# liruihui/SP-GAN

Hardware: AMD Instinct MI355X
Metric: G+D train-step shapes/sec @2048 pts, bs=32 per GPU (WGAN-GP) (higher is better)
Workload: dtype f32; 1 GPU; BASELINE configs[1]: Chair-shaped synthetic clouds, 2048 pts, per-GPU batch 32, WGAN + gradient penalty (lambda 10), 1 D-step + 1 G-step, Adam(1e-4, (0.5,0.99)), k=10; one latent per shape (default noise_generator) handed over un-tiled [b,1,128]; global_batch=32, n_points=2048, parallelism=dp1

## Files before the change

### include/spgan_hip.h

```cpp
#ifndef SPGAN_HIP_H
#define SPGAN_HIP_H

#include <stddef.h>
#include <stdint.h>

#ifdef __cplusplus
extern "C" {
#endif

typedef void* spgan_stream_t;

#define SPGAN_OK 0
#define SPGAN_EINVAL (-22)
#define SPGAN_ECOMM (-70)

int spgan_version(void);
const char* spgan_arch(void);


int spgan_knn(const float* x_pm, int B, int N, int C, int k, int mode, int32_t* idx, spgan_stream_t s);

size_t spgan_knn_ws_bytes(int B, int N, int C, int k, int mode);
int spgan_knn_ws(const float* x_pm, int B, int N, int C, int k, int mode, int32_t* idx, void* ws, size_t ws_bytes, spgan_stream_t s);

// ... 179 lines not shown
size_t spgan_colreduce_ws_bytes(int M, int C, int G);
int spgan_colstats_finalize(const float* partials, int groups, int tiles_per_group, int C, int G, int mode,
                            int tile_rows , float* out0, float* out1, spgan_stream_t s);
int spgan_colstats_finalize_bn(const float* partials, int tiles, int C, int G, int tile_rows, const float* gamma, const float* beta,
                               float eps, float momentum, float* running_mean, float* running_var, float* scale, float* shift,
                               float* invstd, float* mean_out, spgan_stream_t s);
int spgan_colstats_finalize_bn_groups(const float* partials, int groups, int tiles_per_group, int C, int G, int tile_rows, const float* gamma,
                                      const float* beta, float eps, float momentum, float* running_mean, float* running_var, float* out,
                                      spgan_stream_t s);
int spgan_colstats_finalize_bn2(const float* partials, int tiles, int C, int G, int tile_rows, int split, const float* gammaA,
                                const float* betaA, float* rmeanA, float* rvarA, const float* gammaB, const float* betaB, float* rmeanB,
                                float* rvarB, float eps, float momentum, int count_rep, float* out4, spgan_stream_t s);
int spgan_colstats(const float* X, int ldx, int M, int C, int G, float slope, float* out_mean, float* out_var,
                   float* ws, size_t ws_bytes, spgan_stream_t s);
int spgan_colsum(const float* X, int ldx, int M, int C, int G, float* out, float* ws, size_t ws_bytes, spgan_stream_t s);

int spgan_bn_prepare(const float* mean, const float* var, const float* gamma, const float* beta, int C,
                     int count, float eps, float momentum, int training,
                     float* running_mean, float* running_var,
                     float* scale, float* shift, float* invstd, float* mean_used, spgan_stream_t s);
int spgan_bn_bwd_apply(const float* g, const float* y, int ld, int M, int C, const float* mean, const float* invstd,
                       const float* gamma, const float* sums, int count, float* dy, spgan_stream_t s);
int spgan_bn_bwd_apply2(const float* g, const float* g2, const float* g2scale, const float* y, int M, int C, const float* mean,
                        const float* invstd, const float* gamma, const float* sums, int count, float* dy, spgan_stream_t s);

int spgan_maxpool(const float* y, int ld, int B, int N, int C, const float* scale, const float* shift, float slope,
                  float* out, int32_t* argmax, spgan_stream_t s);

int spgan_edge_wcat(const float* Ww0 , const float* Wx , int H, int F, int C, float* Wcat, float* WcatT, spgan_stream_t s);
int spgan_conv_out_weight_pm(const float* w, int F, int k, float* Wo, float* WoT, spgan_stream_t s);
int spgan_edge_wcat_bwd(const float* dWcat, int H, int F, int C, float* dWw0, float* dWx, spgan_stream_t s);
int spgan_edge_stats_tile_rows(int k);
int spgan_edge_stats(const float* PQR, int ld, const int32_t* idx, int M, int k, int H, int F, const float* b1, const float* bx,
                     float* partials, spgan_stream_t s);
int spgan_edge_attend_fwd(const float* h2pre, const float* sc2, const float* sh2, const float* PQR, int ld, int H, int F,
                          const int32_t* idx, int M, int k, const float* bx, const float* scx, const float* shx, float slope,
                          float* T, spgan_stream_t s);
int spgan_edge_attend_fwd_h(const void* h2pre, int h2_half, const float* sc2, const float* sh2, const float* PQR, int ld, int H, int F,
                            const int32_t* idx, int M, int k, const float* bx, const float* scx, const float* shx, float slope, uint16_t* T_f16,
                            spgan_stream_t s);
int spgan_edge_attend_bwd_b(const uint16_t* dT_bf16, const void* h2pre, int h2_half, const float* sc2, const float* sh2, const float* mean2,
                            const float* inv2, const float* PQR, int ld, int H, int F, const int32_t* idx, int M, int k, const float* bx,
                            const float* scx, const float* shx, const float* meanx, const float* invx, float slope, uint16_t* g2_bf16,
                            uint16_t* gy_bf16, float* partials, spgan_stream_t s);
int spgan_edge_scatter_b(const float* g1, const uint16_t* gy_bf16, const float* PQR, int ld, int H, int F, const int32_t* idx,
                         const int32_t* rowptr, const int32_t* src, int M, int k, const float* b1, const float* mean1, const float* inv1,
                         const float* gam1, const float* sums1, const float* bx, const float* meanx, const float* invx, const float* gamx,
                         const float* sumsx, float* dPQR, spgan_stream_t s);
int spgan_edge_attend_bwd_tile_points(void);
int spgan_edge_attend_bwd(const float* dT, const float* h2pre, const float* sc2, const float* sh2, const float* mean2,
                          const float* inv2, const float* PQR, int ld, int H, int F, const int32_t* idx, int M, int k,
                          const float* bx, const float* scx, const float* shx, const float* meanx, const float* invx,
                          float slope, float* g2, float* gy, float* partials, spgan_stream_t s);
int spgan_edge_scatter(const float* g1, const float* gy, const float* PQR, int ld, int H, int F, const int32_t* idx,
                       const int32_t* rowptr, const int32_t* src, int M, int k, const float* b1, const float* mean1,
                       const float* inv1, const float* gam1, const float* sums1, const float* bx, const float* meanx,
                       const float* invx, const float* gamx, const float* sumsx, float* dPQR, spgan_stream_t s);

int spgan_adain_fwd(const float* x, int M, int C, int N, float slope, const float* imean, const float* ivar, float eps,
                    const float* gb, float* out, spgan_stream_t s);
int spgan_adain_bwd1(const float* dout, const float* x, int M, int C, int N, float slope, const float* imean, const float* ivar,
                     float eps, const float* gb, int ld_gamma, long x_shape_stride, float* dgb, float* partials, spgan_stream_t s);
int spgan_adain_bwd2(const float* dout, const float* x, int M, int C, int N, float slope, const float* imean, const float* ivar,
                     float eps, const float* gb, int ld_gamma, long x_shape_stride, const float* S0, const float* S1, float* dx,
                     spgan_stream_t s);

int spgan_pool_bwd_stats(const float* gpool, const float* pooled, const int32_t* argmax, const float* y, int ld, const float* mean,
                         const float* invstd, float slope, int B, int C, float* gval, float* sums , spgan_stream_t s);
int spgan_pool_bwd_stats_prep(const float* gpool, const float* pooled, const int32_t* argmax, const float* y, int ld, const float* mean,
                              const float* invstd, float slope, int B, int C, const float* gamma, int count, float* gval, float* sums ,
                              float* alpha, float* beta, float* cg, spgan_stream_t s);
int spgan_bn_bwd_apply_sparse(const float* gval, const int32_t* argmax, const float* y, int ld, int M, int C, int N,
                              const float* mean, const float* invstd, const float* gamma, const float* sums, int count, float* dy,
                              spgan_stream_t s);
int spgan_maxpool_bwd_add(const float* dpool, const int32_t* argmax, int B, int C, float* dst, int ld, spgan_stream_t s);
int spgan_tanh_bwd(const float* dy, const float* y, size_t n, float* out, spgan_stream_t s);
int spgan_act_bwd(const float* dy, const float* y, size_t n, int act, float slope, float* out, spgan_stream_t s);
int spgan_scatter_rows(const float* val, const int32_t* argmax, int B, int C, int M, float* out, spgan_stream_t s);
int spgan_gather_rows(const float* src, int ld, const int32_t* argmax, int B, int C, float* out, spgan_stream_t s);

int spgan_bn_dbl_stats(const float* u, const float* y, const float* gz, int M, int C, const float* mean, const float* invstd,
                       float* partials, spgan_stream_t s);
int spgan_bn_dbl_apply(const float* u, const float* y, const float* gz, int M, int C, const float* mean, const float* invstd,
                       const float* scale, const float* shift, float slope, const float* gamma, const float* S1, const float* U0,
                       const float* U1, float* q, float* xbar, spgan_stream_t s);
int spgan_gan_loss(int mode, int which, const float* d_real, const float* d_fake, const float* real_label, const float* fake_label,
                   int B, float* out5, float* g_real, float* g_fake, spgan_stream_t s);
int spgan_lerp_rows(const float* real, const float* fake, const float* alpha, int B, size_t L, float* out, spgan_stream_t s);
int spgan_gp_penalty_fwd(const float* g, int B, size_t L, float gamma, float lambda, float* norms, float* loss, spgan_stream_t s);
int spgan_gp_penalty_bwd(const float* g, const float* norms, int B, size_t L, float gamma, float lambda, const float* upstream,
                         float* v, spgan_stream_t s);
int spgan_gp_penalty_fwd_bwd(const float* g, int B, size_t L, float gamma, float lambda, float* norms, float* loss, const float* loss_add,
                             float* loss_total, float* v, spgan_stream_t s);
int spgan_square_distance(const float* src, const float* dst, int B, int N, int M, int C, float* out, spgan_stream_t s);
int spgan_index_points(const float* points, const int64_t* idx, int B, int N, int C, int S, float* out, spgan_stream_t s);
int spgan_farthest_point_sample(const float* xyz, int B, int N, int npoint, const int64_t* start, int64_t* out, float* dist_ws,
                                spgan_stream_t s);
int spgan_query_ball_point(float radius, int nsample, const float* xyz, const float* new_xyz, int B, int N, int S, int C,
                           int64_t* out, spgan_stream_t s);
int spgan_knn_point(int nsample, const float* xyz, const float* new_xyz, int B, int N, int S, int C, int64_t* out, spgan_stream_t s);
int spgan_group_concat(const float* xyz, const float* center, const float* feat, const int64_t* idx, int B, int N, int S, int K,
                       int C, int D, float* out, spgan_stream_t s);
int spgan_gather_csr(const int64_t* idx, int B, int S, int N, int32_t* rowptr, int32_t* src, int32_t* bad, spgan_stream_t s);
int spgan_scatter_slots(const float* dout, int ld, int col0, int C, const int32_t* rowptr, const int32_t* src, int BN, float* dpoints,
                        spgan_stream_t s);
int spgan_group_center_bwd(const float* dout, int ld, int Q, int K, int C, float* dcenter, spgan_stream_t s);
// ... 330 lines not shown
```

### sp-gan_amd/csrc/edge.hip

```cpp
#include <stdlib.h>
#include "common.hpp"

namespace {

__device__ __forceinline__ int xcd_block() {
  const int per = gridDim.x >> 3;
  return (int)(blockIdx.x & 7) * per + (int)(blockIdx.x >> 3);
}
inline int grid8(long n) { return (int)((n + 7) / 8 * 8); }

__global__ void edge_wcat_kernel(const float* __restrict__ Ww0, const float* __restrict__ Wx, int H, int F, int C, float* __restrict__ Wcat,
                                 float* __restrict__ WcatT) {
  const int t = blockIdx.x * blockDim.x + threadIdx.x;
  if (t >= (H + 2 * F) * C) return;
  const int row = t / C, c = t % C;
  float v;
  if (row < H) v = Ww0[row * C + c];
  else if (row < H + F) v = Wx[(row - H) * 2 * C + C + c];
  else v = Wx[(row - H - F) * 2 * C + c] - Wx[(row - H - F) * 2 * C + C + c];
  Wcat[t] = v;
  if (WcatT) WcatT[c * (H + 2 * F) + row] = v;
}
__global__ void conv_out_weight_pm_kernel(const float* __restrict__ w, int F, int k, float* __restrict__ Wo, float* __restrict__ WoT) {
  const int t = blockIdx.x * blockDim.x + threadIdx.x;
  if (t >= F * F * k) return;
  const int o = t / (k * F), q = t % (k * F), r = q / F, c = q % F;
  const float v = w[((size_t)o * F + c) * k + r];
  Wo[t] = v;
  if (WoT) WoT[(size_t)q * F + o] = v;
}
__global__ void edge_wcat_bwd_kernel(const float* __restrict__ dWcat, int H, int F, int C, float* __restrict__ dWw0, float* __restrict__ dWx) {
  const int t = blockIdx.x * blockDim.x + threadIdx.x;
  if (t < H * C) dWw0[t] = dWcat[t];
  if (t < F * C) {
    const int f = t / C, c = t % C;
    const float dq = dWcat[(H + f) * C + c], dr = dWcat[(H + F + f) * C + c];
    dWx[f * 2 * C + c] = dr;
    dWx[f * 2 * C + C + c] = dq - dr;
  }
}

constexpr int ES_PT = 32;

__device__ __forceinline__ float edge_pre(const float* __restrict__ PQR, int ld, int H, int F, int c, int i, int j, float bias) {
  if (c < H) return (PQR[(size_t)j * ld + c] - PQR[(size_t)i * ld + c]) + bias;
  const int f = c - H;
  return (PQR[(size_t)i * ld + H + F + f] + PQR[(size_t)j * ld + H + f]) + bias;
}

template <int KT>
__global__ __launch_bounds__(256) void edge_stats_kernel(const float* __restrict__ PQR, int ld, const int32_t* __restrict__ idx, int M, int k_,
                                                         int H, int F, const float* __restrict__ b1, const float* __restrict__ bx,
                                                         float* __restrict__ part) {
  constexpr int KU = KT > 0 ? KT : 1;
  const int k = KT > 0 ? KT : k_;
  __shared__ float red[4][64];
  const int lane = threadIdx.x & 63, w = __builtin_amdgcn_readfirstlane(threadIdx.x >> 6);
  const int bxid = xcd_block();
  const int p0 = bxid * ES_PT;
  if (p0 >= M) return;
  const int np = min(ES_PT, M - p0);
  const int CH = H + F;
// ... 251 lines not shown
      const float rden = 1.0f / den;
#pragma unroll
      for (int r = 0; r < K; ++r) {
        const float yv = lrelu_f(fmaf((Ri[q] + qv[r][q]) + bb[q], ax[q], cx[q]), slope);
        z[r][q] = yv * (z[r][q] * rden);
      }
    }
#pragma unroll
    for (int r = 0; r < K; ++r) {
      if (TH) stv_h<VEC>(reinterpret_cast<_Float16*>(T) + ((size_t)i * K + r) * F + f, z[r]);
      else stv<VEC>(T + ((size_t)i * K + r) * F + f, z[r]);
    }
  }
}

template <int K, int VEC, int TB = 0, int HH = 0>
__global__ __launch_bounds__(256) void edge_attend_bwd_k_kernel(
    const float* __restrict__ dT, const float* __restrict__ h2, const float* __restrict__ sc2, const float* __restrict__ sh2,
    const float* __restrict__ mean2, const float* __restrict__ inv2, const float* __restrict__ PQR, int ld, int H, int F,
    const int32_t* __restrict__ idx, int M, const float* __restrict__ bx, const float* __restrict__ scx, const float* __restrict__ shx,
    const float* __restrict__ meanx, const float* __restrict__ invx, float slope, float* __restrict__ g2, float* __restrict__ gy,
    float* __restrict__ part) {
  __shared__ float red[4][4][64 * VEC];
  const int lane = threadIdx.x & 63, w = threadIdx.x >> 6;
  const int bxid = xcd_block();
  if (bxid * EB_PT >= M) return;
  for (int f0 = 0; f0 < F; f0 += 64 * VEC) {
    const int f = f0 + lane * VEC;
    const bool ok = f < F;
    float s0[VEC], s1[VEC], s2[VEC], s3[VEC];
#pragma unroll
    for (int q = 0; q < VEC; ++q) s0[q] = s1[q] = s2[q] = s3[q] = 0.f;
    if (ok) {
      float a2[VEC], c2[VEC], ax[VEC], cx[VEC], bb[VEC], m2[VEC], i2[VEC], mxm[VEC], ixv[VEC];
      ldv<VEC>(sc2 + f, a2); ldv<VEC>(sh2 + f, c2); ldv<VEC>(scx + f, ax); ldv<VEC>(shx + f, cx); ldv<VEC>(bx + f, bb);
      ldv<VEC>(mean2 + f, m2); ldv<VEC>(inv2 + f, i2); ldv<VEC>(meanx + f, mxm); ldv<VEC>(invx + f, ixv);
      for (int pp = 0; pp < EB_PT / 4; ++pp) {
        const int i = __builtin_amdgcn_readfirstlane(bxid * EB_PT + pp * 4 + w);
        if (i >= M) break;
        float Ri[VEC];
        ldv<VEC>(PQR + (size_t)i * ld + H + F + f, Ri);
        float hp[K][VEC], d[K][VEC], yp[K][VEC];
#pragma unroll
        for (int r = 0; r < K; ++r) {
          const int j = __builtin_amdgcn_readfirstlane(idx[(size_t)i * K + r]);
          if (HH) ldv_h<VEC>(reinterpret_cast<const _Float16*>(h2) + ((size_t)i * K + r) * F + f, hp[r]);
          else ldv<VEC>(h2 + ((size_t)i * K + r) * F + f, hp[r]);
          if (TB) ldv_b<VEC>(reinterpret_cast<const __bf16*>(dT) + ((size_t)i * K + r) * F + f, d[r]);
          else ldv<VEC>(dT + ((size_t)i * K + r) * F + f, d[r]);
          ldv<VEC>(PQR + (size_t)j * ld + H + f, yp[r]);
        }
        float o2[K][VEC], oy[K][VEC];
#pragma unroll
        for (int q = 0; q < VEC; ++q) {
          float e[K], mx = -INFINITY;
#pragma unroll
          for (int r = 0; r < K; ++r) {
            e[r] = lrelu_f(fmaf(hp[r][q], a2[q], c2[q]), slope);
            mx = fmaxf(mx, e[r]);
          }
          float den = 0.f;
#pragma unroll
          for (int r = 0; r < K; ++r) {
            e[r] = expf(e[r] - mx);
            den += e[r];
          }
          const float rden = 1.0f / den;
          float dot = 0.f;
#pragma unroll
          for (int r = 0; r < K; ++r) {
            yp[r][q] = (Ri[q] + yp[r][q]) + bb[q];
            e[r] *= rden;
            const float yv = lrelu_f(fmaf(yp[r][q], ax[q], cx[q]), slope);
            dot = fmaf(d[r][q] * yv, e[r], dot);
          }
#pragma unroll
          for (int r = 0; r < K; ++r) {
            const float z2 = fmaf(hp[r][q], a2[q], c2[q]);
            const float zy = fmaf(yp[r][q], ax[q], cx[q]);
            const float yv = lrelu_f(zy, slope);
            const float ds = e[r] * (d[r][q] * yv - dot);
            const float v2 = ds * lrelu_mask(z2, slope);
            const float vy = d[r][q] * e[r] * lrelu_mask(zy, slope);
            o2[r][q] = v2; oy[r][q] = vy;
            s0[q] += v2;
            s1[q] = fmaf(v2, (hp[r][q] - m2[q]) * i2[q], s1[q]);
            s2[q] += vy;
            s3[q] = fmaf(vy, (yp[r][q] - mxm[q]) * ixv[q], s3[q]);
          }
        }
#pragma unroll
        for (int r = 0; r < K; ++r) {
          if (TB) stv_b<VEC>(reinterpret_cast<__bf16*>(g2) + ((size_t)i * K + r) * F + f, o2[r]);
          else stv<VEC>(g2 + ((size_t)i * K + r) * F + f, o2[r]);
          if (TB) stv_b<VEC>(reinterpret_cast<__bf16*>(gy) + ((size_t)i * K + r) * F + f, oy[r]);
          else stv<VEC>(gy + ((size_t)i * K + r) * F + f, oy[r]);
        }
      }
    }
#pragma unroll
    for (int q = 0; q < VEC; ++q) {
      red[0][w][lane * VEC + q] = s0[q]; red[1][w][lane * VEC + q] = s1[q];
      red[2][w][lane * VEC + q] = s2[q]; red[3][w][lane * VEC + q] = s3[q];
    }
    __syncthreads();
    for (int c = threadIdx.x; c < 64 * VEC; c += 256) {
      const int ff = f0 + c;
      if (ff < F) {
        float* o = part + (size_t)bxid * (2 * F) * 2;
        o[(size_t)ff * 2 + 0] = (red[0][0][c] + red[0][1][c]) + (red[0][2][c] + red[0][3][c]);
        o[(size_t)ff * 2 + 1] = (red[2][0][c] + red[2][1][c]) + (red[2][2][c] + red[2][3][c]);
        o[(size_t)(F + ff) * 2 + 0] = (red[1][0][c] + red[1][1][c]) + (red[1][2][c] + red[1][3][c]);
        o[(size_t)(F + ff) * 2 + 1] = (red[3][0][c] + red[3][1][c]) + (red[3][2][c] + red[3][3][c]);
      }
    }
    __syncthreads();
  }
}

#ifndef SPGAN_SCATTER_CHUNK
#define SPGAN_SCATTER_CHUNK 16
#endif
constexpr int SCH = SPGAN_SCATTER_CHUNK;
template <int KT, int GB = 0>
__global__ __launch_bounds__(256) void edge_scatter_kernel(
    const float* __restrict__ g1, const float* __restrict__ gy, const float* __restrict__ PQR, int ld, int H, int F,
    const int32_t* __restrict__ idx, const int32_t* __restrict__ rowptr, const int32_t* __restrict__ src, int M, int k_,
    const float* __restrict__ b1, const float* __restrict__ mean1, const float* __restrict__ inv1, const float* __restrict__ gam1,
    const float* __restrict__ sums1, const float* __restrict__ bx, const float* __restrict__ meanx, const float* __restrict__ invx,
    const float* __restrict__ gamx, const float* __restrict__ sumsx, float rE, float* __restrict__ dPQR) {
  constexpr int KU = KT > 0 ? KT : 1;
  const int k = KT > 0 ? KT : k_;
  const int lane = threadIdx.x & 63;
  const int j = __builtin_amdgcn_readfirstlane(xcd_block() * 4 + (threadIdx.x >> 6));
  if (j >= M) return;
  auto ldgy = [&](size_t off) -> float {
    return GB ? (float)reinterpret_cast<const __bf16*>(gy)[off] : gy[off];
  };
  const int t0 = rowptr[j], t1 = rowptr[j + 1];
  int jo[KU];
  if (KT > 0) {
#pragma unroll
    for (int r = 0; r < KU; ++r) jo[r] = idx[j * KT + r];
// ... 220 lines not shown
```

### sp-gan_amd/spgan/_lib.py

```python
from __future__ import annotations

import ctypes as C
import os

_HERE = os.path.dirname(os.path.abspath(__file__))
LIB_PATH = os.path.join(_HERE, "libspgan_hip.so")

c_f32p = C.c_void_p
c_i32p = C.c_void_p
c_i64p = C.c_void_p
stream_t = C.c_void_p


class ColTail(C.Structure):
    _fields_ = [("enabled", C.c_int), ("mode", C.c_int),
                ("out0", c_f32p), ("out1", c_f32p),
                ("gamma", c_f32p), ("beta", c_f32p), ("rmean", c_f32p), ("rvar", c_f32p),
                ("scale", c_f32p), ("shift", c_f32p), ("invstd", c_f32p), ("mean_out", c_f32p),
                ("eps", C.c_float), ("momentum", C.c_float), ("count_rep", C.c_int)]


class GemmNTArgs(C.Structure):
    _fields_ = [
        ("A", c_f32p), ("lda", C.c_int),
# ... 150 lines not shown
SIGNATURES = {
    "spgan_version": (I, []),
    "spgan_arch": (C.c_char_p, []),
    "spgan_knn": (I, [P, I, I, I, I, I, P, P]),
    "spgan_knn_ws_bytes": (SZ, [I, I, I, I, I]),
    "spgan_knn_ws": (I, [P, I, I, I, I, I, P, P, SZ, P]),
    "spgan_csr_build": (I, [P, I, I, I, P, P, P]),
    "spgan_edge_features_cm": (I, [P, P, I, I, I, I, P, P]),
    "spgan_idx_to_local64": (I, [P, I, I, I, P, P]),
    "spgan_idx_from_local64": (I, [P, I, I, I, P, P]),
    "spgan_cm_to_pm": (I, [P, I, I, I, P, P]),
    "spgan_pm_to_cm": (I, [P, I, I, I, P, P]),
    "spgan_concat2": (I, [P, I, P, I, I, P, P]),
    "spgan_gemm_nt": (I, [C.POINTER(GemmNTArgs), P]),
    "spgan_gemm_nt_col_blocks": (I, [C.POINTER(GemmNTArgs)]),
    "spgan_split_bf16x3_image_bytes": (C.c_size_t, [I, I]),
    "spgan_split_bf16x3_image": (I, [P, I, I, I, P, P]),
    "spgan_gemm_nt_uses_w_image": (I, [C.POINTER(GemmNTArgs)]),
    "spgan_gemm_nt_owns_columns": (I, [C.POINTER(GemmNTArgs)]),
    "spgan_pool_finalize": (I, [P, P, I, I, I, P, P, F, P, P, P, P]),
    "spgan_pool_finalize_groups": (I, [P, P, I, I, I, P, P, I, I, F, P, P, P, I, P]),
    "spgan_pool_zero_scale_yarg": (I, [P, I, P, I, P, P, P, F, I, I, I, I, I, P, I, I, P, P]),
    "spgan_gemm_tn_ws_bytes": (SZ, [I, I, I]),
    "spgan_gemm_tn_ws_bytes_lp": (SZ, [I, I, I, I]),
    "spgan_gemm_tn_splits_lp": (I, [I, I, I, I]),
    "spgan_gemm_tn": (I, [C.POINTER(GemmTNArgs), P]),
    "spgan_gemm_tn_skinny_multi": (I, [C.POINTER(GemmTNArgs), I, P]),
    "spgan_sparse_rows_nt": (I, [P, P, I, I, I, P, I, I, P, I, P]),
    "spgan_sparse_rows_tn": (I, [P, P, I, I, I, P, I, I, P, P, F, P, I, P]),
    "spgan_affine_act": (I, [P, I, SZ, I, P, P, F, P, P]),
    "spgan_rowscale_outer": (I, [P, I, I, I, P, P, P, P, P, I, I, P]),
    "spgan_colreduce_ws_bytes": (SZ, [I, I, I]),
    "spgan_colstats_finalize": (I, [P, I, I, I, I, I, I, P, P, P]),
    "spgan_colstats_finalize_bn": (I, [P, I, I, I, I, P, P, F, F, P, P, P, P, P, P, P]),
    "spgan_colstats_finalize_bn_groups": (I, [P, I, I, I, I, I, P, P, F, F, P, P, P, P]),
    "spgan_colstats_finalize_bn2": (I, [P, I, I, I, I, I, P, P, P, P, P, P, P, P, F, F, I, P, P]),
    "spgan_colstats": (I, [P, I, I, I, I, F, P, P, P, SZ, P]),
    "spgan_colsum": (I, [P, I, I, I, I, P, P, SZ, P]),
    "spgan_bn_prepare": (I, [P, P, P, P, I, I, F, F, I, P, P, P, P, P, P, P]),
    "spgan_bn_bwd_apply": (I, [P, P, I, I, I, P, P, P, P, I, P, P]),
    "spgan_bn_bwd_apply2": (I, [P, P, P, P, I, I, P, P, P, P, I, P, P]),
    "spgan_maxpool": (I, [P, I, I, I, I, P, P, F, P, P, P]),
    "spgan_edge_wcat": (I, [P, P, I, I, I, P, P, P]),
    "spgan_conv_out_weight_pm": (I, [P, I, I, P, P, P]),
    "spgan_edge_wcat_bwd": (I, [P, I, I, I, P, P, P]),
    "spgan_edge_stats_tile_rows": (I, [I]),
    "spgan_edge_stats": (I, [P, I, P, I, I, I, I, P, P, P, P]),
    "spgan_edge_attend_fwd": (I, [P, P, P, P, I, I, I, P, I, I, P, P, P, F, P, P]),
    "spgan_edge_attend_fwd_h": (I, [P, I, P, P, P, I, I, I, P, I, I, P, P, P, F, P, P]),
    "spgan_edge_attend_bwd_b": (I, [P, P, I, P, P, P, P, P, I, I, I, P, I, I, P, P, P, P, P, F, P, P, P, P]),
    "spgan_gemm_nt_y16_ok": (I, [P]),
    "spgan_edge_attend_bwd_tile_points": (I, []),
    "spgan_edge_attend_bwd": (I, [P, P, P, P, P, P, P, I, I, I, P, I, I, P, P, P, P, P, F, P, P, P, P]),
    "spgan_edge_scatter_b": (I, [P, P, P, I, I, I, P, P, P, I, I, P, P, P, P, P, P, P, P, P, P, P, P]),
    "spgan_edge_scatter": (I, [P, P, P, I, I, I, P, P, P, I, I, P, P, P, P, P, P, P, P, P, P, P, P]),
    "spgan_adain_fwd": (I, [P, I, I, I, F, P, P, F, P, P, P]),
    "spgan_adain_bwd1": (I, [P, P, I, I, I, F, P, P, F, P, I, C.c_long, P, P, P]),
    "spgan_adain_bwd2": (I, [P, P, I, I, I, F, P, P, F, P, I, C.c_long, P, P, P, P]),
    "spgan_pool_bwd_stats": (I, [P, P, P, P, I, P, P, F, I, I, P, P, P]),
    "spgan_pool_bwd_stats_prep": (I, [P, P, P, P, I, P, P, F, I, I, P, I, P, P, P, P, P, P]),
    "spgan_bn_bwd_apply_sparse": (I, [P, P, P, I, I, I, I, P, P, P, P, I, P, P]),
    "spgan_maxpool_bwd_add": (I, [P, P, I, I, P, I, P]),
    "spgan_tanh_bwd": (I, [P, P, SZ, P, P]),
    "spgan_act_bwd": (I, [P, P, SZ, I, F, P, P]),
    "spgan_scatter_rows": (I, [P, P, I, I, I, P, P]),
    "spgan_gather_rows": (I, [P, I, P, I, I, P, P]),
    "spgan_bn_dbl_stats": (I, [P, P, P, I, I, P, P, P, P]),
    "spgan_bn_dbl_apply": (I, [P, P, P, I, I, P, P, P, P, F, P, P, P, P, P, P, P]),
    "spgan_bn_dbl_coeffs": (I, [P, P, P, P, P, P, P, I, I, P, P]),
    "spgan_bn_dbl_phaseb": (I, [P, P, P, P, P, I, P, P, P]),
    "spgan_bn_dbl_phaseb_sums": (I, [P, P, P, P, P, P, P, P, P, I, I, P, P, P]),
    "spgan_gather_rowdot": (I, [P, I, P, P, I, I, I, I, P, P]),
    "spgan_rowdot": (I, [P, I, P, I, I, I, P, P]),
    "spgan_dbl_top_dots": (I, [P, I, P, P, I, P, I, P, I, I, I, P, P, P, P]),
    "spgan_bn_dbl_pool": (I, [P, P, P, P, P, P, P, P, P, P, P, P, I, I, I, F, P, P, P, P]),
    "spgan_sparse_bn_prep": (I, [P, P, P, P, P, I, I, I, P, P, P, P]),
    "spgan_col_scale_add": (I, [P, P, P, I, I, P, P]),
    "spgan_gan_loss": (I, [I, I, P, P, P, P, I, P, P, P, P]),
    "spgan_lerp_rows": (I, [P, P, P, I, SZ, P, P]),
    "spgan_gp_penalty_fwd": (I, [P, I, SZ, F, F, P, P, P]),
    "spgan_gp_penalty_bwd": (I, [P, P, I, SZ, F, F, P, P, P]),
    "spgan_gp_penalty_fwd_bwd": (I, [P, I, SZ, F, F, P, P, P, P, P, P]),
    "spgan_square_distance": (I, [P, P, I, I, I, I, P, P]),
    "spgan_index_points": (I, [P, P, I, I, I, I, P, P]),
    "spgan_farthest_point_sample": (I, [P, I, I, I, P, P, P, P]),
    "spgan_query_ball_point": (I, [F, I, P, P, I, I, I, I, P, P]),
    "spgan_knn_point": (I, [I, P, P, I, I, I, I, P, P]),
    "spgan_group_concat": (I, [P, P, P, P, I, I, I, I, I, I, P, P]),
    "spgan_wt_diag_w": (I, [P, I, I, I, P, P, P, P, I, P, P]),
    "spgan_collapse_prep": (I, [C.POINTER(CollapsePrepArgs), P]),
    "spgan_wgrad_collapse": (I, [C.POINTER(WgradCollapseArgs), P]),
    "spgan_wgrad_collapse_multi": (I, [C.POINTER(WgradCollapseArgs), I, P]),
    "spgan_gemm_dual_wgs": (I, [I, I, I, I]),
    "spgan_gemm_dual_rows_per_wg": (I, [I, I, I]),
    "spgan_gemm_dual": (I, [C.POINTER(GemmDualArgs), P]),
    "spgan_gemm_dual_multi": (I, [C.POINTER(GemmDualArgs), I, P]),
    "spgan_colstats_finalize_multi": (I, [C.POINTER(ColFinalizeArgs), I, P]),
    "spgan_pool_bwd_stats_prep_multi": (I, [C.POINTER(PoolBwdArgs), I, P]),
    "spgan_gather_csr": (I, [P, I, I, I, P, P, P, P]),
    "spgan_scatter_slots": (I, [P, I, I, I, P, P, I, P, P]),
    "spgan_group_center_bwd": (I, [P, I, I, I, I, P, P]),
    "spgan_edge_features_cm_bwd": (I, [P, P, P, I, I, I, I, P, P]),
    "spgan_three_nn": (I, [P, P, I, I, I, P, P, P]),
    "spgan_three_interpolate": (I, [P, P, P, I, I, I, I, I, P, I, I, P, P]),
    "spgan_three_interpolate_bwd": (I, [P, I, I, I, P, I, P, P, I, P, P]),
    "spgan_group_max": (I, [P, I, I, I, I, P, P, F, P, P, P]),
# ... 177 lines not shown
```

### sp-gan_amd/spgan/nets.py

```python
from __future__ import annotations

import os
import weakref
from typing import Dict, List, Optional, Tuple

import torch

from . import adain_epi, ops

Tensor = torch.Tensor
NEG = 0.01
NEG_2 = 0.2
ZERO_GRAD = 0


def _w2(w: Tensor) -> Tensor:
    return w.view(w.shape[0], w.shape[1])


_T_CACHE: Dict[Tuple[int, Tuple[int, ...]], tuple] = {}


def owned(p: Tensor) -> Tensor:
    d = p.detach()
    if isinstance(p, torch.nn.Parameter):
        d._spgan_owner = weakref.ref(p)
    return d


def _owner(w: Tensor):
    base = w._base if w._base is not None else w
    if isinstance(base, torch.nn.Parameter):
        return base
    ref = getattr(base, "_spgan_owner", None)
    return ref() if ref is not None else None


def _t(w: Tensor) -> Tensor:
    owner = _owner(w)
    if owner is None:
        return w.t().contiguous()
    key = (w.data_ptr(), tuple(w.shape))
    stamp = (ops.WEIGHTS_EPOCH[0], owner._version)
    hit = _T_CACHE.get(key)
    if hit is not None and hit[2]() is owner:
        if hit[0] == stamp:
            return hit[1]
        _refresh_transposes(owner)
        hit = _T_CACHE.get(key)
        if hit is not None and hit[0] == stamp:
            return hit[1]
    t = w.t().contiguous()
    _T_CACHE[key] = (stamp, t, weakref.ref(owner), (tuple(w.shape), tuple(w.stride()), w.storage_offset()))
    return t


_COLS_CACHE: Dict[tuple, tuple] = {}


def _cols_from(w: Tensor, c: int) -> Tensor:
    owner = _owner(w)
# ... 818 lines not shown
                      count_rep: int = 1, bn_repeats: int = 1, out: Optional[Tensor] = None):
    if bn_repeats > 1 and training:
        with ops.bn_momentum(1.0 - (1.0 - ops.BN_MOMENTUM) ** bn_repeats):
            out, ctx = edgeblock_forward(P, bufs, pre, x, idx, B, N, training, update_running, count_rep, 1, out=out)
        if bufs is not None and update_running:
            for _ in range(bn_repeats - 1):
                for bn in (".conv_w.1", ".conv_x.1", ".conv_w.4"):
                    _count_bn_call(bufs, pre + bn)
        return out, ctx
    return _edgeblock_forward(P, bufs, pre, x, idx, B, N, training, update_running, count_rep, out=out)


def _edgeblock_forward(P, bufs, pre: str, x: Tensor, idx: Tensor, B: int, N: int, training: bool = True, update_running: bool = True,
                       count_rep: int = 1, out: Optional[Tensor] = None):
    M, C = x.shape
    k = idx.shape[1]
    Ww0 = P[pre + ".conv_w.0.weight"]; Wx = P[pre + ".conv_x.0.weight"]
    H, F_ = Ww0.shape[0], Wx.shape[0]
    b1, bx = P[pre + ".conv_w.0.bias"], P[pre + ".conv_x.0.bias"]
    Wcat, WcatT = ops.edge_wcat(_w2(Ww0), _w2(Wx), transposed=True)
    PQR = ops.gemm_nt(x, Wcat)
    E = M * k
    if training:
        run = lambda n: (bufs[n + ".running_mean"], bufs[n + ".running_var"]) if (bufs is not None and update_running) else (None, None)
        bn1, bnx = ops.edge_stats_bn(PQR, idx, b1, bx,
                                     (P[pre + ".conv_w.1.weight"], P[pre + ".conv_w.1.bias"]) + run(pre + ".conv_w.1"),
                                     (P[pre + ".conv_x.1.weight"], P[pre + ".conv_x.1.bias"]) + run(pre + ".conv_x.1"), count_rep)
        if bufs is not None and update_running:
            _count_bn_call(bufs, pre + ".conv_w.1"); _count_bn_call(bufs, pre + ".conv_x.1")
    else:
        bn1 = _bn_train(None, None, P, bufs, pre + ".conv_w.1", E, False, False)
        bnx = _bn_train(None, None, P, bufs, pre + ".conv_x.1", E, False, False)
    W2, b2 = _w2(P[pre + ".conv_w.3.weight"]), P[pre + ".conv_w.3.bias"]
    s16 = ops.storage16(E, F_, k) and _lazy_ok(E, F_)
    h2pre, bn2 = _gemm_bn(PQR[:, :H], W2, b2, P, bufs, pre + ".conv_w.4", E, training, update_running, pro=(bn1[0], bn1[1], NEG), edge=(idx, b1),
                          **({"count_rep": count_rep} if training and count_rep > 1 else {}), **({"out_half": True} if s16 else {}))
    T = ops.edge_attend_fwd(h2pre, bn2[0], bn2[1], PQR, idx, bx, bnx[0], bnx[1], NEG, half=s16)
    Wo, WoT = conv_out_weight_pm(P[pre + ".conv_out.weight"])
    out = ops.gemm_nt(T, Wo, P[pre + ".conv_out.bias"], out=out)
    ctx = dict(x=x, idx=idx, B=B, N=N, PQR=PQR, Wcat=Wcat, WcatT=WcatT, WoT=WoT, bn1=bn1, bnx=bnx, bn2=bn2, h2pre=h2pre, T=T, Wo=Wo, H=H, F=F_, k=k, training=training)
    return out, ctx


def edgeblock_backward(P, pre: str, ctx, dout: Tensor, csr: Tuple[Tensor, Tensor], need_dx: bool = True):
    x, idx, PQR, H, F_, k = ctx["x"], ctx["idx"], ctx["PQR"], ctx["H"], ctx["F"], ctx["k"]
    M = x.shape[0]
    E = M * k
    bn1, bnx, bn2 = ctx["bn1"], ctx["bnx"], ctx["bn2"]
    b1, bx = P[pre + ".conv_w.0.bias"], P[pre + ".conv_x.0.bias"]
    g: Dict[str, Tensor] = {}
    dout = dout.contiguous()
    gwo, g[pre + ".conv_out.bias"] = ops.gemm_tn(dout, ctx["T"], with_colsum=True, defer=True)
    g[pre + ".conv_out.weight"] = conv_out_weight_grad_from_pm(gwo, F_, k)
    dT = ops.gemm_nt(dout, ctx["WoT"], out_bf16=ctx["T"].dtype == torch.float16)
    g2, gy, sums2, sumsy = ops.edge_attend_bwd(dT, ctx["h2pre"], bn2[0], bn2[1], bn2[3], bn2[2], PQR, idx, bx, bnx[0], bnx[1], bnx[3], bnx[2], NEG)
    g[pre + ".conv_w.4.weight"] = sums2[F_:]; g[pre + ".conv_w.4.bias"] = sums2[:F_]
    g[pre + ".conv_x.1.weight"] = sumsy[F_:]; g[pre + ".conv_x.1.bias"] = sumsy[:F_]
    if not ctx["training"]:
        sums2 = torch.zeros_like(sums2); sumsy = torch.zeros_like(sumsy)
    dh2 = _bn_bwd(g2, ctx["h2pre"], bn2[3], bn2[2], P[pre + ".conv_w.4.weight"], sums2, E)
    W2 = _w2(P[pre + ".conv_w.3.weight"])
    if ctx["training"] and ops.gemm_dual_ok(dh2, W2, PQR[:, :H], edge=(idx, b1)):
        dW3, g1, s10, s11 = ops.gemm_dual(dh2, W2, PQR[:, :H], bn1[0], bn1[1], bn1[3], bn1[2], NEG, edge=(idx, b1))
        g[pre + ".conv_w.3.weight"] = dW3.view_as(P[pre + ".conv_w.3.weight"])
    else:
        g[pre + ".conv_w.3.weight"] = ops.gemm_tn(dh2, PQR[:, :H], pro=(bn1[0], bn1[1], NEG), edge=(idx, b1), defer=True).view_as(P[pre + ".conv_w.3.weight"])
        g1, s10, s11 = ops.gemm_nt_bnbwd(dh2, _t(W2), PQR[:, :H], bn1[0], bn1[1], bn1[3], bn1[2], NEG, edge=(idx, b1))
    g[pre + ".conv_w.3.bias"] = ZERO_GRAD if ctx["training"] else ops.colsum(_dense(dh2))[0]
    g[pre + ".conv_w.1.weight"] = s11; g[pre + ".conv_w.1.bias"] = s10
    sums1 = _cat2(s10, s11) if ctx["training"] else torch.zeros(2 * H, device=x.device)
    dPQR = ops.edge_scatter(g1, gy, PQR, idx, csr[0], csr[1], b1, bn1[3], bn1[2], P[pre + ".conv_w.1.weight"], sums1,
                            bx, bnx[3], bnx[2], P[pre + ".conv_x.1.weight"], sumsy)
    dWcat = ops.gemm_tn(dPQR, x)
    dW0, dWx = ops.edge_wcat_bwd(dWcat, H, F_)
    g[pre + ".conv_w.0.weight"] = dW0.view_as(P[pre + ".conv_w.0.weight"])
    g[pre + ".conv_x.0.weight"] = dWx.view_as(P[pre + ".conv_x.0.weight"])
    g[pre + ".conv_w.0.bias"] = ZERO_GRAD
    g[pre + ".conv_x.0.bias"] = ZERO_GRAD
    dx = ops.gemm_nt(dPQR, ctx["WcatT"]) if need_dx else None
    return dx, g


def adain_forward(P, pre: str, x: Tensor, style: Tensor, N: int, slope: float = 1.0, fused: Optional[dict] = None):
    Ws, bs = _w2(P[pre + ".style.weight"]), P[pre + ".style.bias"]
    M = style.shape[0]
    if fused is not None and adain_epi.usable(x, style, Ws, N):
        if x.shape[0] != M:
            imean, ivar = adain_epi.shared_stats(x, slope, M // N)
        else:
            imean, ivar = ops.colstats(x, N, slope)
            imean = imean.contiguous(); ivar = ivar.contiguous()
        pool = bool(fused.get("pool")) and adain_epi.can_pool(M, N)
        r0 = fused.get("gamma_row0", 0)
        out, gamma, rec = adain_epi.forward(x, style, Ws, bs, N, slope, imean, ivar, gamma_row0=r0, pool=pool)
        return out, dict(x=x, style=style, gb=None, gamma=gamma, gamma_row0=r0, imean=imean, ivar=ivar, N=N, slope=slope, pool=rec)
    if x.shape[0] != M:
        x = x.repeat(M // N, 1)
    gb = ops.gemm_nt(style, Ws, bs)
    imean, ivar = ops.colstats(x, N, slope)
    imean = imean.contiguous(); ivar = ivar.contiguous()
    out = ops.adain_fwd(x, N, slope, imean, ivar, gb)
    return out, dict(x=x, style=style, gb=gb, imean=imean, ivar=ivar, N=N, slope=slope)


def adain_backward(P, pre: str, ctx, dout: Tensor, need_dx: bool = True, need_dstyle: bool = True, need_dparams: bool = True,
                   dstyle_addend: Optional[Tensor] = None):
    if ctx.get("gamma") is not None:
        dx, dgb = adain_epi.backward(dout.contiguous(), ctx["x"], ctx["N"], ctx["slope"], ctx["imean"], ctx["ivar"], ctx["gamma"])
# ... 234 lines not shown
```

Baseline: 3649 shapes/s.

## Fuse dT GEMM into edge-attention backward kernel via MFMA tiles

Adds a fused HIP kernel that computes dT = dout·WoT with f32 MFMA into registers and immediately applies the edge-attention softmax/leaky-ReLU backward, writing g2/gy and partial BN sums. The goal is to skip writing and re-reading the [M*k, F] dT intermediate and save one kernel launch. It only applies for k=10, F=128, f32 with the f16 MFMA path off, and falls back to the old GEMM plus backward path otherwise. The shared elementwise math moves into a header, with fp contraction disabled to keep results matching the old path.

```diff
diff --git a/include/spgan_hip.h b/include/spgan_hip.h
--- a/include/spgan_hip.h
+++ b/include/spgan_hip.h
@@ -255,6 +255,11 @@
                           const float* inv2, const float* PQR, int ld, int H, int F, const int32_t* idx, int M, int k,
                           const float* bx, const float* scx, const float* shx, const float* meanx, const float* invx,
                           float slope, float* g2, float* gy, float* partials, spgan_stream_t s);
+int spgan_edge_attend_bwd_dt_selected(const float* dout, int ldo, const float* WoT, int ldw, int M, int k, int F, int tile_hint);
+int spgan_edge_attend_bwd_dt(const float* dout, int ldo, const float* WoT, int ldw, const float* h2pre, const float* sc2, const float* sh2,
+                             const float* mean2, const float* inv2, const float* PQR, int ld, int H, int F, const int32_t* idx, int M, int k,
+                             const float* bx, const float* scx, const float* shx, const float* meanx, const float* invx, float slope,
+                             float* g2, float* gy, float* partials, spgan_stream_t s);
 int spgan_edge_scatter(const float* g1, const float* gy, const float* PQR, int ld, int H, int F, const int32_t* idx,
                        const int32_t* rowptr, const int32_t* src, int M, int k, const float* b1, const float* mean1,
                        const float* inv1, const float* gam1, const float* sums1, const float* bx, const float* meanx,
diff --git a/sp-gan_amd/csrc/edge.hip b/sp-gan_amd/csrc/edge.hip
--- a/sp-gan_amd/csrc/edge.hip
+++ b/sp-gan_amd/csrc/edge.hip
@@ -1,13 +1,8 @@
 #include <stdlib.h>
 #include "common.hpp"
+#include "edge_attend.hpp"
 
 namespace {
-
-__device__ __forceinline__ int xcd_block() {
-  const int per = gridDim.x >> 3;
-  return (int)(blockIdx.x & 7) * per + (int)(blockIdx.x >> 3);
-}
-inline int grid8(long n) { return (int)((n + 7) / 8 * 8); }
 
 __global__ void edge_wcat_kernel(const float* __restrict__ Ww0, const float* __restrict__ Wx, int H, int F, int C, float* __restrict__ Wcat,
                                  float* __restrict__ WcatT) {
@@ -365,43 +360,8 @@
         }
         float o2[K][VEC], oy[K][VEC];
 #pragma unroll
-        for (int q = 0; q < VEC; ++q) {
-          float e[K], mx = -INFINITY;
-#pragma unroll
-          for (int r = 0; r < K; ++r) {
-            e[r] = lrelu_f(fmaf(hp[r][q], a2[q], c2[q]), slope);
-            mx = fmaxf(mx, e[r]);
-          }
-          float den = 0.f;
-#pragma unroll
-          for (int r = 0; r < K; ++r) {
-            e[r] = expf(e[r] - mx);
-            den += e[r];
-          }
-          const float rden = 1.0f / den;
-          float dot = 0.f;
-#pragma unroll
-          for (int r = 0; r < K; ++r) {
-            yp[r][q] = (Ri[q] + yp[r][q]) + bb[q];
-            e[r] *= rden;
-            const float yv = lrelu_f(fmaf(yp[r][q], ax[q], cx[q]), slope);
-            dot = fmaf(d[r][q] * yv, e[r], dot);
-          }
-#pragma unroll
-          for (int r = 0; r < K; ++r) {
-            const float z2 = fmaf(hp[r][q], a2[q], c2[q]);
-            const float zy = fmaf(yp[r][q], ax[q], cx[q]);
-            const float yv = lrelu_f(zy, slope);
-            const float ds = e[r] * (d[r][q] * yv - dot);
-            const float v2 = ds * lrelu_mask(z2, slope);
-            const float vy = d[r][q] * e[r] * lrelu_mask(zy, slope);
-            o2[r][q] = v2; oy[r][q] = vy;
-            s0[q] += v2;
-            s1[q] = fmaf(v2, (hp[r][q] - m2[q]) * i2[q], s1[q]);
-            s2[q] += vy;
-            s3[q] = fmaf(vy, (yp[r][q] - mxm[q]) * ixv[q], s3[q]);
-          }
-        }
+        for (int q = 0; q < VEC; ++q)
+          edge_attend_bwd_elem<K, VEC, VEC == 1>(q, hp, d, yp, Ri, a2, c2, ax, cx, bb, m2, i2, mxm, ixv, slope, o2, oy, s0, s1, s2, s3);
 #pragma unroll
         for (int r = 0; r < K; ++r) {
           if (TB) stv_b<VEC>(reinterpret_cast<__bf16*>(g2) + ((size_t)i * K + r) * F + f, o2[r]);
diff --git a/sp-gan_amd/csrc/edge_attend.hpp b/sp-gan_amd/csrc/edge_attend.hpp
--- /dev/null
+++ b/sp-gan_amd/csrc/edge_attend.hpp
@@ -0,0 +1,53 @@
+#pragma once
+#include "common.hpp"
+
+__device__ __forceinline__ int xcd_block() {
+  const int per = gridDim.x >> 3;
+  return (int)(blockIdx.x & 7) * per + (int)(blockIdx.x >> 3);
+}
+inline int grid8(long n) { return (int)((n + 7) / 8 * 8); }
+
+template <int K, int VEC, bool FUSED_SUMS>
+__device__ __forceinline__ void edge_attend_bwd_elem(int q, const float (&hp)[K][VEC], const float (&d)[K][VEC], float (&yp)[K][VEC],
+                                                     const float (&Ri)[VEC], const float (&a2)[VEC], const float (&c2)[VEC], const float (&ax)[VEC],
+                                                     const float (&cx)[VEC], const float (&bb)[VEC], const float (&m2)[VEC], const float (&i2)[VEC],
+                                                     const float (&mxm)[VEC], const float (&ixv)[VEC], float slope, float (&o2)[K][VEC],
+                                                     float (&oy)[K][VEC], float (&s0)[VEC], float (&s1)[VEC], float (&s2)[VEC], float (&s3)[VEC]) {
+#pragma clang fp contract(off)
+  float e[K], mx = -INFINITY;
+#pragma unroll
+  for (int r = 0; r < K; ++r) {
+    e[r] = lrelu_f(fmaf(hp[r][q], a2[q], c2[q]), slope);
+    mx = fmaxf(mx, e[r]);
+  }
+  float den = 0.f;
+#pragma unroll
+  for (int r = 0; r < K; ++r) {
+    e[r] = expf(e[r] - mx);
+    den += e[r];
+  }
+  const float rden = 1.0f / den;
+  float dot = 0.f;
+#pragma unroll
+  for (int r = 0; r < K; ++r) {
+    yp[r][q] = (Ri[q] + yp[r][q]) + bb[q];
+    e[r] *= rden;
+    const float yv = lrelu_f(fmaf(yp[r][q], ax[q], cx[q]), slope);
+    dot = fmaf(d[r][q] * yv, e[r], dot);
+  }
+#pragma unroll
+  for (int r = 0; r < K; ++r) {
+    const float z2 = fmaf(hp[r][q], a2[q], c2[q]);
+    const float zy = fmaf(yp[r][q], ax[q], cx[q]);
+    const float yv = lrelu_f(zy, slope);
+    const float ds = e[r] * fmaf(d[r][q], yv, -dot);
+    const float k2 = lrelu_mask(z2, slope), ky = lrelu_mask(zy, slope), de = d[r][q] * e[r];
+    const float v2 = ds * k2;
+    const float vy = de * ky;
+    o2[r][q] = v2; oy[r][q] = vy;
+    s0[q] = FUSED_SUMS ? fmaf(ds, k2, s0[q]) : s0[q] + v2;
+    s1[q] = fmaf(v2, (hp[r][q] - m2[q]) * i2[q], s1[q]);
+    s2[q] = FUSED_SUMS ? fmaf(de, ky, s2[q]) : s2[q] + vy;
+    s3[q] = fmaf(vy, (yp[r][q] - mxm[q]) * ixv[q], s3[q]);
+  }
+}
diff --git a/sp-gan_amd/csrc/edge_dt.hip b/sp-gan_amd/csrc/edge_dt.hip
--- /dev/null
+++ b/sp-gan_amd/csrc/edge_dt.hip
@@ -0,0 +1,180 @@
+#include <stdlib.h>
+#include "edge_attend.hpp"
+#include "gemm_wide.hpp"
+
+typedef float f32x16 __attribute__((ext_vector_type(16)));
+
+namespace {
+
+constexpr int DK = 10, DF = 128;
+constexpr int DP = 32;
+constexpr int DKT = 32, DLW = DKT + 2;
+constexpr int DLA = DF + 2;
+constexpr int DNKT = DF / DKT;
+constexpr size_t DT_LDS = ((size_t)DP * DLA + 2 * DF * DLW + DP * DK) * sizeof(float);
+
+__device__ __forceinline__ int row_point(int i) {
+  const int lh = (i >> 2) & 1, v = (i & 3) + 4 * (i >> 3);
+  return 4 * (v >> 1) + 2 * lh + (v & 1);
+}
+
+__global__ __launch_bounds__(256, 2) void edge_attend_bwd_dt_kernel(
+    const float* __restrict__ dout, int ldo, const float* __restrict__ WoT, int ldw, const float* __restrict__ h2,
+    const float* __restrict__ sc2, const float* __restrict__ sh2, const float* __restrict__ mean2, const float* __restrict__ inv2,
+    const float* __restrict__ PQR, int ld, int H, const int32_t* __restrict__ idx, int M, const float* __restrict__ bx,
+    const float* __restrict__ scx, const float* __restrict__ shx, const float* __restrict__ meanx, const float* __restrict__ invx, float slope,
+    float* __restrict__ g2, float* __restrict__ gy, float* __restrict__ part) {
+  constexpr int THREADS = 256, SLOTS = 4, RPP = 32;
+  extern __shared__ __attribute__((aligned(16))) float smem[];
+  float* As = smem;
+  float* Bs = smem + DP * DLA;
+  int* sidx = reinterpret_cast<int*>(Bs + 2 * DF * DLW);
+  const int tid = threadIdx.x, lane = tid & 63, w = tid >> 6;
+  const int l31 = lane & 31, lh = lane >> 5;
+  const int bxid = xcd_block();
+  const int i0 = bxid * DP;
+  if (i0 >= M) return;
+
+#pragma unroll
+  for (int s = 0; s < 4; ++s) {
+    const int q = tid + s * THREADS, row = q >> 5, c4 = (q & 31) * 4;
+    const int i = i0 + row_point(row);
+    const float4 v = *reinterpret_cast<const float4*>(dout + (size_t)i * ldo + c4);
+    float* a = As + row * DLA + c4;
+    *reinterpret_cast<float2*>(a) = make_float2(v.x, v.y);
+    *reinterpret_cast<float2*>(a + 2) = make_float2(v.z, v.w);
+  }
+  for (int t = tid; t < DP * DK; t += THREADS) sidx[t] = idx[(size_t)i0 * DK + t];
+
+  f32x16 acc[DK];
+#pragma unroll
+  for (int r = 0; r < DK; ++r)
+#pragma unroll
+    for (int v = 0; v < 16; ++v) acc[r][v] = 0.f;
+
+  float4 rb[SLOTS];
+  const int lrow = tid >> 3, lc4 = (tid & 7) * 4;
+  auto gload = [&](int r, int kt) {
+#pragma unroll
+    for (int i = 0; i < SLOTS; ++i)
+      rb[i] = *reinterpret_cast<const float4*>(WoT + (size_t)(r * DF + lrow + RPP * i) * ldw + kt * DKT + lc4);
+  };
+  auto sstore = [&](int buf) {
+    float* b = Bs + buf * DF * DLW + lrow * DLW + lc4;
+#pragma unroll
+    for (int i = 0; i < SLOTS; ++i) {
+      *reinterpret_cast<float2*>(b + i * RPP * DLW) = make_float2(rb[i].x, rb[i].y);
+      *reinterpret_cast<float2*>(b + i * RPP * DLW + 2) = make_float2(rb[i].z, rb[i].w);
+    }
+  };
+  const float* afrag = As + l31 * DLA + 2 * lh;
+  const float* bfrag = Bs + (w * 32 + l31) * DLW + 2 * lh;
+
+  const int f = w * 32 + l31;
+  float hp[2][DK][1], yp[2][DK][1], Ri[2][1];
+  auto fetch = [&](int v) {
+    const int p = 4 * (v >> 1) + 2 * lh + (v & 1);
+    const size_t i = (size_t)(i0 + p);
+    Ri[v & 1][0] = PQR[i * ld + H + DF + f];
+#pragma unroll
+    for (int r = 0; r < DK; ++r) {
+      const int j = sidx[p * DK + r];
+      hp[v & 1][r][0] = h2[(i * DK + r) * DF + f];
+      yp[v & 1][r][0] = PQR[(size_t)j * ld + H + f];
+    }
+  };
+
+  gload(0, 0);
+  sstore(0);
+  __syncthreads();
+#pragma unroll
+  for (int r = 0; r < DK; ++r) {
+#pragma unroll
+    for (int kt = 0; kt < DNKT; ++kt) {
+      const int s = r * DNKT + kt, buf = s & 1;
+      if (s + 1 < DK * DNKT) gload((s + 1) / DNKT, (s + 1) % DNKT);
+      if (s == DK * DNKT - 2) fetch(0);
+      float2 af[DKT / 4], bf[DKT / 4];
+#pragma unroll
+      for (int kk = 0; kk < DKT / 4; ++kk) {
+        af[kk] = *reinterpret_cast<const float2*>(afrag + kt * DKT + kk * 4);
+        bf[kk] = *reinterpret_cast<const float2*>(bfrag + buf * DF * DLW + kk * 4);
+      }
+#pragma unroll
+      for (int kk = 0; kk < DKT / 4; ++kk) {
+        acc[r] = __builtin_amdgcn_mfma_f32_32x32x2f32(af[kk].x, bf[kk].x, acc[r], 0, 0, 0);
+        acc[r] = __builtin_amdgcn_mfma_f32_32x32x2f32(af[kk].y, bf[kk].y, acc[r], 0, 0, 0);
+      }
+      __builtin_amdgcn_sched_group_barrier(0x020, 32, 0);
+      __builtin_amdgcn_sched_group_barrier(0x100, 8, 0);
+      __builtin_amdgcn_sched_group_barrier(0x008, 16, 0);
+      __builtin_amdgcn_sched_barrier(0);
+      if (s + 1 < DK * DNKT) sstore(buf ^ 1);
+      __syncthreads();
+    }
+  }
+
+  const float a2[1] = {sc2[f]}, c2[1] = {sh2[f]}, ax[1] = {scx[f]}, cx[1] = {shx[f]}, bb[1] = {bx[f]}, m2[1] = {mean2[f]}, i2[1] = {inv2[f]},
+              mxm[1] = {meanx[f]}, ixv[1] = {invx[f]};
+  float sums[2][4][1] = {};
+#pragma unroll
+  for (int v = 0; v < 16; ++v) {
+    if (v + 1 < 16) fetch(v + 1);
+    __builtin_amdgcn_sched_barrier(0);
+    const int p = 4 * (v >> 1) + 2 * lh + (v & 1);
+    const size_t e0 = ((size_t)(i0 + p) * DK) * DF + f;
+    float d[DK][1], o2[DK][1], oy[DK][1];
+#pragma unroll
+    for (int r = 0; r < DK; ++r) d[r][0] = acc[r][v];
+    auto& s = sums[v & 1];
+    edge_attend_bwd_elem<DK, 1, false>(0, hp[v & 1], d, yp[v & 1], Ri[v & 1], a2, c2, ax, cx, bb, m2, i2, mxm, ixv, slope, o2, oy, s[0], s[1], s[2],
+                                       s[3]);
+#pragma unroll
+    for (int r = 0; r < DK; ++r) {
+      g2[e0 + (size_t)r * DF] = o2[r][0];
+      gy[e0 + (size_t)r * DF] = oy[r][0];
+    }
+    __builtin_amdgcn_sched_barrier(0);
+  }
+  float tot[4];
+#pragma unroll
+  for (int n = 0; n < 4; ++n) {
+    const float t = sums[0][n][0] + sums[1][n][0];
+    tot[n] = t + __shfl_xor(t, 32);
+  }
+  if (lh == 0) {
+    float* o = part + (size_t)bxid * (2 * DF) * 2;
+    o[(size_t)f * 2 + 0] = tot[0];
+    o[(size_t)f * 2 + 1] = tot[2];
+    o[(size_t)(DF + f) * 2 + 0] = tot[1];
+    o[(size_t)(DF + f) * 2 + 1] = tot[3];
+  }
+}
+
+inline bool al(const void* q, uintptr_t a) { return (reinterpret_cast<uintptr_t>(q) & (a - 1)) == 0; }
+
+}
+
+extern "C" int spgan_edge_attend_bwd_dt_selected(const float* dout, int ldo, const float* WoT, int ldw, int M, int k, int F, int tile_hint) {
+  if (!dout || !WoT || k != DK || F != DF || M <= 0 || M % DP) return 0;
+  spgan_gemm_nt_args a = {};
+  a.A = dout; a.lda = ldo; a.W = WoT; a.ldw = ldw;
+  a.Y = const_cast<float*>(dout); a.ldy = k * F;
+  a.M = M; a.N = k * F; a.K = F;
+  a.a_mode = SPGAN_A_PLAIN; a.epi_mode = SPGAN_EPI_LINEAR; a.mfma_f16 = 0; a.tile_hint = tile_hint;
+  return spgan_nt_wide_selected(a) ? 1 : 0;
+}
+
+extern "C" int spgan_edge_attend_bwd_dt(const float* dout, int ldo, const float* WoT, int ldw, const float* h2pre, const float* sc2,
+                                        const float* sh2, const float* mean2, const float* inv2, const float* PQR, int ld, int H, int F,
+                                        const int32_t* idx, int M, int k, const float* bx, const float* scx, const float* shx, const float* meanx,
+                                        const float* invx, float slope, float* g2, float* gy, float* partials, spgan_stream_t s_) {
+  SPGAN_CHECK_ARG(dout && WoT && h2pre && sc2 && sh2 && mean2 && inv2 && PQR && idx && bx && scx && shx && meanx && invx && g2 && gy && partials);
+  SPGAN_CHECK_ARG(k == DK && F == DF && M > 0 && M % DP == 0 && H >= 0 && ld >= H + 2 * F);
+  SPGAN_CHECK_ARG(ldo >= F && ldo % 4 == 0 && ldw >= F && ldw % 4 == 0 && al(dout, 16) && al(WoT, 16));
+  SPGAN_CHECK_ARG(al(h2pre, 4) && al(sc2, 4) && al(sh2, 4) && al(mean2, 4) && al(inv2, 4) && al(PQR, 4) && al(idx, 4) && al(bx, 4) && al(scx, 4) &&
+                  al(shx, 4) && al(meanx, 4) && al(invx, 4) && al(g2, 4) && al(gy, 4) && al(partials, 4));
+  hipLaunchKernelGGL(edge_attend_bwd_dt_kernel, dim3(grid8(M / DP)), dim3(256), DT_LDS, (hipStream_t)s_, dout, ldo, WoT, ldw, h2pre, sc2, sh2, mean2,
+                     inv2, PQR, ld, H, idx, M, bx, scx, shx, meanx, invx, slope, g2, gy, partials);
+  return spgan_launch_status();
+}
diff --git a/sp-gan_amd/spgan/_lib.py b/sp-gan_amd/spgan/_lib.py
--- a/sp-gan_amd/spgan/_lib.py
+++ b/sp-gan_amd/spgan/_lib.py
@@ -226,6 +226,8 @@
     "spgan_gemm_nt_y16_ok": (I, [P]),
     "spgan_edge_attend_bwd_tile_points": (I, []),
     "spgan_edge_attend_bwd": (I, [P, P, P, P, P, P, P, I, I, I, P, I, I, P, P, P, P, P, F, P, P, P, P]),
+    "spgan_edge_attend_bwd_dt_selected": (I, [P, I, P, I, I, I, I, I]),
+    "spgan_edge_attend_bwd_dt": (I, [P, I, P, I, P, P, P, P, P, P, I, I, I, P, I, I, P, P, P, P, P, F, P, P, P, P]),
     "spgan_edge_scatter_b": (I, [P, P, P, I, I, I, P, P, P, I, I, P, P, P, P, P, P, P, P, P, P, P, P]),
     "spgan_edge_scatter": (I, [P, P, P, I, I, I, P, P, P, I, I, P, P, P, P, P, P, P, P, P, P, P, P]),
     "spgan_adain_fwd": (I, [P, I, I, I, F, P, P, F, P, P, P]),
diff --git a/sp-gan_amd/spgan/edge_dt.py b/sp-gan_amd/spgan/edge_dt.py
--- /dev/null
+++ b/sp-gan_amd/spgan/edge_dt.py
@@ -0,0 +1,81 @@
+from __future__ import annotations
+
+from typing import Optional
+
+import torch
+
+from . import _lib, ops
+from ._lib import check
+from .ops import _f32, _finalize, _i32, _ld, _p, _pqr, _rowmajor2d, _s, _vec
+
+Tensor = torch.Tensor
+
+ENABLED = [True]
+LAUNCHES = [0]
+
+
+class route:
+
+    def __init__(self, on: bool):
+        self.on = bool(on)
+
+    def __enter__(self):
+        self.prev = ENABLED[0]
+        ENABLED[0] = self.on
+
+    def __exit__(self, *exc):
+        ENABLED[0] = self.prev
+
+
+def edge_attend_bwd_dt_selected(dout: Tensor, WoT: Tensor, k: int, F_: int) -> bool:
+    if not (dout.is_cuda and WoT.is_cuda) or dout.dtype != torch.float32 or WoT.dtype != torch.float32 or ops._MFMA_F16[0] != 0:
+        return False
+    if dout.dim() != 2 or WoT.dim() != 2 or dout.stride(1) != 1 or WoT.stride(1) != 1 or dout.shape[1] != F_ or tuple(WoT.shape) != (k * F_, F_):
+        return False
+    return bool(_lib.load().spgan_edge_attend_bwd_dt_selected(_p(dout), _ld(dout), _p(WoT), _ld(WoT), dout.shape[0], k, F_, ops._NT_TILE_HINT[0]))
+
+
+def edge_attend_bwd_dt(dout: Tensor, WoT: Tensor, h2pre: Tensor, sc2, sh2, mean2, inv2, PQR: Tensor, idx: Tensor, bx, scx, shx, meanx, invx,
+                       slope: float, _part_out: Optional[list] = None):
+    F_ = bx.numel()
+    H = PQR.shape[1] - 2 * F_
+    _pqr(PQR, H, F_); _i32(idx, "idx")
+    M_, k = idx.shape
+    _rowmajor2d(dout, "dout"); _rowmajor2d(WoT, "WoT"); _f32(h2pre, "h2pre", 2)
+    if dout.shape != (M_, F_) or WoT.shape != (k * F_, F_) or not h2pre.is_contiguous() or h2pre.numel() != M_ * k * F_:
+        raise ValueError("dout [M,F], WoT [k*F,F] and a contiguous h2pre with M*k*F elements expected")
+    lib = _lib.load()
+    tp = lib.spgan_edge_attend_bwd_tile_points()
+    tiles = (M_ + tp - 1) // tp
+    g2 = torch.empty((M_ * k, F_), dtype=torch.float32, device=PQR.device)
+    gy = torch.empty((M_ * k, F_), dtype=torch.float32, device=PQR.device)
+    part = torch.empty((tiles, 2 * F_, 2), dtype=torch.float32, device=PQR.device)
+    v = lambda t, n: _p(_vec(t, F_, n))
+    check(lib.spgan_edge_attend_bwd_dt(_p(dout), _ld(dout), _p(WoT), _ld(WoT), _p(h2pre), v(sc2, "sc2"), v(sh2, "sh2"), v(mean2, "mean2"),
+                                       v(inv2, "inv2"), _p(PQR), PQR.shape[1], H, F_, _p(idx), M_, k, v(bx, "bx"), v(scx, "scx"), v(shx, "shx"),
+                                       v(meanx, "meanx"), v(invx, "invx"), float(slope), _p(g2), _p(gy), _p(part), _s()),
+          "edge_attend_bwd_dt", M=M_, k=k, F=F_)
+    if _part_out is not None:
+        _part_out.append(part)
+    s0, s1 = _finalize(part, 1, tiles, 2 * F_, tiles * tp, 1, tp)
+    return g2, gy, s0[0], s1[0]
+
+
+ops.edge_attend_bwd_dt = edge_attend_bwd_dt
+ops.edge_attend_bwd_dt_selected = edge_attend_bwd_dt_selected
+
+
+def usable(dout: Tensor, WoT: Tensor, T: Tensor, h2pre: Tensor, PQR: Tensor, k: int, F_: int) -> bool:
+    if not ENABLED[0] or k != 10 or F_ != 128:
+        return False
+    for t in (dout, WoT, T, h2pre, PQR):
+        if not isinstance(t, torch.Tensor) or not t.is_cuda or t.dtype != torch.float32:
+            return False
+    if not (h2pre.is_contiguous() and PQR.is_contiguous()):
+        return False
+    return edge_attend_bwd_dt_selected(dout, WoT, k, F_)
+
+
+def backward(dout: Tensor, WoT: Tensor, h2pre: Tensor, sc2, sh2, mean2, inv2, PQR: Tensor, idx: Tensor, bx, scx, shx, meanx, invx, slope: float):
+    LAUNCHES[0] += 1
+    return edge_attend_bwd_dt(dout, WoT, h2pre, sc2, sh2, mean2, inv2, PQR, idx, bx, scx, shx, meanx, invx, slope)
diff --git a/sp-gan_amd/spgan/nets.py b/sp-gan_amd/spgan/nets.py
--- a/sp-gan_amd/spgan/nets.py
+++ b/sp-gan_amd/spgan/nets.py
@@ -6,7 +6,7 @@
 
 import torch
 
-from . import adain_epi, ops
+from . import adain_epi, edge_dt, ops
 
 Tensor = torch.Tensor
 NEG = 0.01
@@ -931,8 +931,12 @@
     dout = dout.contiguous()
     gwo, g[pre + ".conv_out.bias"] = ops.gemm_tn(dout, ctx["T"], with_colsum=True, defer=True)
     g[pre + ".conv_out.weight"] = conv_out_weight_grad_from_pm(gwo, F_, k)
-    dT = ops.gemm_nt(dout, ctx["WoT"], out_bf16=ctx["T"].dtype == torch.float16)
-    g2, gy, sums2, sumsy = ops.edge_attend_bwd(dT, ctx["h2pre"], bn2[0], bn2[1], bn2[3], bn2[2], PQR, idx, bx, bnx[0], bnx[1], bnx[3], bnx[2], NEG)
+    if edge_dt.usable(dout, ctx["WoT"], ctx["T"], ctx["h2pre"], PQR, k, F_):
+        g2, gy, sums2, sumsy = edge_dt.backward(dout, ctx["WoT"], ctx["h2pre"], bn2[0], bn2[1], bn2[3], bn2[2], PQR, idx, bx, bnx[0], bnx[1],
+                                                bnx[3], bnx[2], NEG)
+    else:
+        dT = ops.gemm_nt(dout, ctx["WoT"], out_bf16=ctx["T"].dtype == torch.float16)
+        g2, gy, sums2, sumsy = ops.edge_attend_bwd(dT, ctx["h2pre"], bn2[0], bn2[1], bn2[3], bn2[2], PQR, idx, bx, bnx[0], bnx[1], bnx[3], bnx[2], NEG)
     g[pre + ".conv_w.4.weight"] = sums2[F_:]; g[pre + ".conv_w.4.bias"] = sums2[:F_]
     g[pre + ".conv_x.1.weight"] = sumsy[F_:]; g[pre + ".conv_x.1.bias"] = sumsy[:F_]
     if not ctx["training"]:
```

Result: faster. 3706 shapes/s, median of 6 (+1.6%).
